# at-cg/PHI

Hardware: AMD Instinct MI355X
Metric: read Gbases/s scored (49-hap MHC graph stand-in synMHC-49); reads resident in HBM, parsing and H2D excluded (higher is better)
Workload: dtype u64

## Files before the change

### phi_amd/csrc/dp_events.hip

```cpp
#include <hip/hip_runtime.h>
#include <type_traits>
#include "phi_kernels.h"

#define NEG (-(1 << 28))
#define NEGK (-(1 << 30))
#define CHK PHI_DP_CHUNK
#define RING PHI_DP_RING
enum { DP_SEQ = 0, DP_ROW = 1, DP_PATH = 2 };

__global__ void __launch_bounds__(256) phi_event_flags_kernel(const int32_t *__restrict__ walk_vtx, int64_t n_entries,
                                                              const int32_t *__restrict__ cvtx, uint8_t *__restrict__ flags)
{
    for (int64_t e = (int64_t)blockIdx.x * blockDim.x + threadIdx.x; e < n_entries; e += (int64_t)gridDim.x * blockDim.x)
        flags[e] = cvtx[walk_vtx[e]] >= 0;
}

__global__ void phi_event_off_kernel(const phi_ent_t *__restrict__ ev_e, int64_t n_ev, const int64_t *__restrict__ walk_off,
                                     int32_t n_walks, int64_t *__restrict__ ev_off)
{
    const int h = blockIdx.x * blockDim.x + threadIdx.x;
    if (h > n_walks) return;
    const int64_t key = walk_off[h];
    int64_t lo = 0, hi = n_ev;
    while (lo < hi) {
// ... 998 lines not shown
        }
        issue(J, min(b + DEPTH, nb - 1));
        __syncthreads();
#pragma unroll
        for (int u = 0; u < U; u++) {
            int32_t best = NEGK;
            if (has_walk) {
                if (live[u]) { const int32_t r = s_diag[p][lx]; if (r > NEGK / 2) best = S[u] + r; }
                {
                    const int32_t o = (live[u] && v[u] == b1[u] && s_n1[p][u][lx] == 1) ? s_b2[p][u][lx] : b1[u];
                    const int32_t kn = s_new[p][lx];
                    if (o > NEGK / 2 && kn > NEGK / 2 && o + kn - dx > best) best = o + kn - dx;
                }
                const int32_t d = max(max(s_part[p][u][0][lx], s_part[p][u][1][lx]), max(s_part[p][u][2][lx], s_part[p][u][3][lx]));
                if (d > NEGK / 2 && d - dx > best) best = d - dx;
                if (with_starts[u]) { const int32_t r = s_start[p][lx]; if (r > NEGK / 2 && r - dx > best) best = r - dx; }
            }
            S[u] = best > NEGK / 2 ? best : NEGK;
        }
    };
    if (x < 64) {
#pragma unroll
        for (int u = 0; u < U; u++) { s_b1[b_lo & 1][u][x] = NONE; s_b2[b_lo & 1][u][x] = NONE; s_n1[b_lo & 1][u][x] = 0; }
    }
    using I0 = std::integral_constant<int, 0>; using I1 = std::integral_constant<int, 1>;
    using I2 = std::integral_constant<int, 2>; using I3 = std::integral_constant<int, 3>;
    issue(I0{}, min(b_lo, nb - 1));
    issue(I1{}, min(b_lo + 1, nb - 1));
    issue(I2{}, min(b_lo + 2, nb - 1));
    issue(I3{}, min(b_lo + 3, nb - 1));
    __syncthreads();
    int32_t b = b_lo;
    for (; b + DEPTH <= nb; b += DEPTH) {
        step(I0{}, b);
        step(I1{}, b + 1);
        step(I2{}, b + 2);
        step(I3{}, b + 3);
    }
    if (b < nb) step(I0{}, b);
    if (b + 1 < nb) step(I1{}, b + 1);
    if (b + 2 < nb) step(I2{}, b + 2);
    if (MODE == 1 && has_walk) {
#pragma unroll
        for (int u = 0; u < U; u++)
            if (unit0 + u <= G.n_walks) seg_row[((int64_t)seg * (G.n_walks + 1) + unit0 + u) * LS + x] = S[u];
    }
}

__global__ void __launch_bounds__(256) phi_seg_chain_kernel(int32_t n_seg, int32_t n_walks, int32_t LS, const int32_t *__restrict__ seg_row,
                                                            int32_t *__restrict__ seg_S)
{
    __shared__ int32_t s_S[256];
    const int x = threadIdx.x;
    int32_t S = NEGK;
    for (int32_t g = 0; g < n_seg; g++) {
        seg_S[(int64_t)g * LS + x] = S;
        s_S[x] = S;
        __syncthreads();
        const int32_t *R = seg_row + (int64_t)g * (n_walks + 1) * LS + x;
        int32_t best = R[(int64_t)n_walks * LS];
#pragma unroll 8
        for (int32_t u = 0; u < n_walks; u++) best = max(best, s_S[u] + R[(int64_t)u * LS]);
        S = best > NEGK / 2 ? best : NEGK;
        __syncthreads();
    }
}

__global__ void __launch_bounds__(256) phi_blk_check_kernel(const int32_t *__restrict__ keys, const int32_t *__restrict__ S, int32_t n_blk,
                                                            int32_t LS, int32_t n_walks, int32_t *__restrict__ bad)
{
    const int64_t n = (int64_t)(n_blk - 1) * LS;
    for (int64_t i = (int64_t)blockIdx.x * blockDim.x + threadIdx.x; i < n; i += (int64_t)gridDim.x * blockDim.x) {
        const int32_t h = (int32_t)(i % LS);
        if (h >= n_walks) continue;
        const int32_t got = keys[i], want = S[i + LS];
        if (got != want && !(got <= NEGK / 2 && want <= NEGK / 2)) { atomicAdd(&bad[0], 1); atomicMin(&bad[1], (int32_t)(i / LS)); }
    }
}

__global__ void __launch_bounds__(256) phi_carry_resolve_kernel(const int32_t *__restrict__ carry, int32_t LS, int32_t b_from, int32_t h,
                                                                int32_t *__restrict__ out)
{
    __shared__ int32_t s_best;
    for (int32_t hi = b_from - 1; hi >= 0; hi -= 256) {
        if (threadIdx.x == 0) s_best = -1;
        __syncthreads();
        const int32_t b = hi - (int32_t)threadIdx.x;
        const int32_t v = b >= 0 ? carry[(int64_t)b * LS + h] : -1;
        if (v >= 0) atomicMax(&s_best, b);
        __syncthreads();
        const int32_t bb = s_best;
        if (bb >= 0) {
            if (b == bb) { out[0] = bb; out[1] = v; }
            return;
        }
        __syncthreads();
    }
    if (threadIdx.x == 0) { out[0] = -1; out[1] = -1; }
}

void phi_launch_blk_classes(hipStream_t st, const PhiBlkClassArgs &G)
{
    if (G.n_blk > 0) hipLaunchKernelGGL(phi_blk_classes_kernel, dim3((unsigned)G.n_blk), dim3(256), 0, st, G);
}
void phi_launch_blk_chain(hipStream_t st, const PhiBlkClassArgs &G, const int32_t *rows, const int32_t *rownew, const int32_t *rowdiag, int32_t *blk_S)
{
    hipLaunchKernelGGL(phi_blk_chain_kernel<0>, dim3(1), dim3(256), 0, st, G, rows, rownew, rowdiag, blk_S, nullptr, nullptr, nullptr);
}
void phi_launch_blk_chain_segments(hipStream_t st, const PhiBlkClassArgs &G, const int32_t *rows, const int32_t *rownew, const int32_t *rowdiag, int32_t *blk_S,
                                   int32_t n_seg, const int32_t *d_seg_lo, int32_t *seg_row, int32_t *seg_S)
{
    const int units = getenv("PHI_DP_CHAIN_UNITS") ? atoi(getenv("PHI_DP_CHAIN_UNITS")) : 3;
// ... 51 lines not shown
```

### phi_amd/csrc/phi_ctx.h

```cpp
#pragma once
#include <stdint.h>
#include <stdarg.h>
#include <stdio.h>
#include <stdlib.h>
#include <algorithm>
#include <atomic>
#include <chrono>
#include <future>
#include <mutex>
#include <string>
#include <thread>
#include <vector>
#include <hip/hip_runtime.h>
#include "../../include/phi_amd.h"
#include "phi_kernels.h"
#include "phi_host_par.h"

struct DevBuf {
    void *p = nullptr;
    size_t cap = 0;
    uint32_t gen = 0;
    template <class T> T *as() const { return reinterpret_cast<T *>(p); }
};

// ... 162 lines not shown
        uint32_t why = 0, first_bad = 0;
    } text;

    struct PhiBamStream {
        bool active = false, failed = false, header_done = false;
        int32_t n_ref = 0;
        uint32_t tile = 0, list_cap = 0, max_tiles = 0, max_rec = 0;
        uint32_t carry_cap = 0, chunk_cap = 0;
        std::vector<unsigned char> h_hdr;
        int64_t fed = 0;
        DevBuf text[2];
        DevBuf bases, roff, sum;
        DevBuf t_first, t_exit, t_status, t_cnt, t_skip, t_list, t_has, t_has_pre, t_use, t_base;
        DevBuf rec_pos, rec_keep, kidx, klen, kseq, krev;
        int slot = 0;
        uint32_t carry_len = 0, carry_at = 0;
        void *h_sum = nullptr;
        hipEvent_t ev_copy = nullptr;
        int64_t one_len = -1;
        int64_t dbg_reads = 0, dbg_bases = 0;
        phi_bam_info info{};
    } bam;

    struct PhiLadder {
        bool collecting = false, have_store = false, have_plan = false;
        int64_t first_ordinal = 0;
        int64_t n_reads = 0, n_bases = 0;
        int64_t one_len = -1;
        DevBuf d_bases, d_off;
        DevBuf d_pbases, d_poff, d_pidx, d_psrc, d_wg, d_tab;
        int64_t band_read0[PHI_LADDER_MAX_LEVELS + 1] = {0}, band_pos[PHI_LADDER_MAX_LEVELS + 1] = {0};
        int32_t scored = 0;
        phi_ladder_info info{};
    } ladder;

    DevBuf d_blk_cnt, d_blk_off, d_flags, d_flags2, d_list, d_list2, d_list3, d_walk_last;
    DevBuf d_sel_off, d_sel_tri;
    DevBuf d_adj_off, d_adj, d_topo_rank, d_cnt_edge, d_walk_err;
    DevBuf d_sa_cnt, d_sa_cur, d_sa_off, d_sa_idx;

    DevBuf d_m_rec, d_m_group, d_g_keys, d_g_rep, d_g_cnt, d_slot_maxcnt, d_slot_multi;
    DevBuf d_a_e1, d_g_off, d_g_span, d_a_weight;
    DevBuf d_dmax, d_bstart, d_top, d_ent, d_word;
    bool dp_dense_ready = false;
    bool dp_events = false;
    int32_t n_k = 0;
    int64_t n_ev = 0;
    std::vector<int32_t> h_cstep, h_kstep;
    std::vector<int32_t> h_k_cut_ok;
    bool dp_blocks = false;
    int32_t n_blk = 0, blk_ring = 1024, blk_max_len = 0;
    std::vector<int32_t> h_blk_lo;
    DevBuf d_blk_lo, d_blk_ev, d_blk_S, d_row_out, d_rowend, d_blk_keys, d_blk_carry, d_cov, d_cov2, d_stepdiff;
    bool dp_cls = false;
    int32_t blk_cls_target = 16;
    bool blk_no_small = false;
    int32_t blk_ls = 64;
    DevBuf d_lane_walk, d_walk_lane, d_coff, d_blk_ncls, d_rownew, d_blk_bad;
    DevBuf d_seg_lo, d_seg_row, d_seg_S;
    DevBuf d_k_rec, d_k_in, d_cvtx, d_ev_e, d_ev_off, d_ev, d_off_end, d_off_start, d_scan_blk, d_scan_blk64, d_scan_blkoff;
    DevBuf d_anchors, d_cov_all, d_cov_w, d_slots, d_slots2, d_segs, d_ctr, d_vmax;
    int64_t n_kept = 0, n_dp = 0;
    bool anchors_host = false;
    PhiAnchorSpan h_kept, h_dp;
    std::vector<PhiAnchorHost> h_dp_own;
    void *h_pin = nullptr;
    size_t h_pin_cap = 0;
    std::future<void> pin_future;
    std::future<int> dp_alloc_future;
    std::vector<uint64_t> h_kept_hash;
    std::vector<int32_t> h_path_vtx, h_path_hap;
    std::vector<int64_t> h_n_minimizers, h_n_anchors;
    phi_result result{};
    bool solved = false;

    bool prof = false;
    std::vector<std::pair<hipEvent_t, hipEvent_t>> prof_events;
    int prof_period = 1;
    uint64_t prof_seq = 0;
    size_t prof_used = 0;
    int64_t prof_bases = 0;
    double prof_ms_done = 0.0;
    int64_t prof_n_done = 0;
};

struct PhiStageTimer {
    bool on;
    const char *what;
    std::chrono::steady_clock::time_point t0;
    explicit PhiStageTimer(const char *w) : on(getenv("PHI_TIMING") != nullptr), what(w), t0(std::chrono::steady_clock::now()) {}
    void lap(const char *stage)
    {
        if (!on) return;
        const auto t1 = std::chrono::steady_clock::now();
        fprintf(stderr, "[phi timing] %s: %-28s %8.3f ms\n", what, stage, std::chrono::duration<double, std::milli>(t1 - t0).count());
        t0 = t1;
    }
};

static inline hipError_t phi_copy_sync(phi_ctx *c, void *dst, const void *src, size_t n, hipMemcpyKind kind)
{
    const hipError_t e = hipMemcpyAsync(dst, src, n, kind, c->stream);
    return e != hipSuccess ? e : hipStreamSynchronize(c->stream);
}
static inline hipError_t phi_memset_sync(phi_ctx *c, void *dst, int v, size_t n)
{
    const hipError_t e = hipMemsetAsync(dst, v, n, c->stream);
// ... 73 lines not shown
```

### phi_amd/csrc/phi_solve.hip

```cpp
#include <stdio.h>
#include <string.h>
#include <algorithm>
#include <map>
#include <set>
#include <unordered_map>
#include "phi_ctx.h"
#include "phi_dev.h"

#define HIPCHK(call) do { int rc_ = phi_hip_check(c, (call), #call); if (rc_) return rc_; } while (0)
#define PHICHK(call) do { int rc_ = (call); if (rc_) return rc_; } while (0)

static bool have_host_walks(const phi_ctx *c) { return (int64_t)c->h_walk_vtx.size() == c->n_entries; }
static int walk_vtx_at(phi_ctx *c, int64_t e, int32_t *v)
{
    if (have_host_walks(c)) { *v = c->h_walk_vtx[(size_t)e]; return PHI_OK; }
    return phi_hip_check(c, phi_copy_sync(c, v, c->d_walk_vtx.as<int32_t>() + e, 4, hipMemcpyDeviceToHost), "walk entry D2H");
}
static int walk_vtx_range(phi_ctx *c, int64_t es, int64_t n, int32_t *dst)
{
    if (have_host_walks(c)) { memcpy(dst, c->h_walk_vtx.data() + es, (size_t)n * 4); return PHI_OK; }
    return phi_hip_check(c, phi_copy_sync(c, dst, c->d_walk_vtx.as<int32_t>() + es, (size_t)n * 4, hipMemcpyDeviceToHost), "walk entries D2H");
}
static int ensure_host_walks(phi_ctx *c)
{
    if (have_host_walks(c)) return PHI_OK;
    if (!c->h_walk_vtx.resize((size_t)c->n_entries)) return phi_fail(c, PHI_ERR_NOMEM, "host allocation failed");
    return phi_hip_check(c, phi_copy_sync(c, c->h_walk_vtx.data(), c->d_walk_vtx.p, (size_t)c->n_entries * 4, hipMemcpyDeviceToHost), "walk entries D2H");
}

struct Seg { int32_t h; int64_t es, ee; };

int phi_host_anchors(phi_ctx *c)
{
    if (c->anchors_host) return PHI_OK;
    const int64_t n = c->n_kept;
    PHICHK(phi_pin_ensure(c, (size_t)std::max<int64_t>(n, 1) * sizeof(PhiAnchorHost)));
    c->h_kept = PhiAnchorSpan{static_cast<PhiAnchorHost *>(c->h_pin), n};
    if (n) HIPCHK(hipMemcpyAsync(c->h_kept.p, c->d_anchors.p, (size_t)n * 12, hipMemcpyDeviceToHost, c->stream));
    HIPCHK(hipStreamSynchronize(c->stream));
    c->h_dp_own.clear();
    c->h_dp = c->h_kept;
    c->anchors_host = true;
    return PHI_OK;
}

static int dp_prepare_blocks(phi_ctx *c, int64_t n_dp)
{
    c->dp_blocks = false;
    c->n_blk = 0;
    c->dp_cls = false;
    if (!c->dp_events || c->n_walks > PHI_DP_EVENT_MAX_WALKS || getenv("PHI_DP_NOBLOCKS") || c->n_k < 4) return PHI_OK;
    const bool cls = c->n_walks > 64;
    c->blk_ls = cls ? 256 : 64;
    const int64_t ne = c->n_entries;
    const int32_t nk = c->n_k;
    PHICHK(phi_dev_ensure(c, c->d_off_end, (size_t)(ne + 3) * 4));
    PHICHK(phi_dev_ensure(c, c->d_off_start, (size_t)(ne + 3) * 4));
    PHICHK(phi_dev_ensure(c, c->d_stepdiff, (size_t)(nk + 2) * 4));
    int32_t *d_a = c->d_off_end.as<int32_t>(), *d_b = c->d_off_start.as<int32_t>();
    HIPCHK(hipMemsetAsync(c->d_stepdiff.p, 0, (size_t)(nk + 2) * 4, c->stream));
    if (getenv("PHI_CUT_COUNTED")) {
        HIPCHK(hipMemsetAsync(d_a, 0, (size_t)(ne + 3) * 4, c->stream));
        phi_launch_cut_cov(c->stream, c->d_a_e1.as<phi_ent_t>(), c->d_g_span.as<uint8_t>(), n_dp, d_a);
        PHICHK(phi_scan(c, d_a, ne + 1, d_b));
        phi_launch_cut_clean(c->stream, d_b, ne, d_a);
    } else {
        phi_launch_cut_clean_direct(c->stream, c->d_g_off.as<int64_t>(), c->d_g_span.as<uint8_t>(), ne, d_a);
    }
    PHICHK(phi_scan(c, d_a, ne + 1, d_b));
    phi_launch_cut_events(c->stream, c->d_ev_e.as<phi_ent_t>(), c->n_ev, c->d_ev_off.as<int64_t>(), c->d_walk_off.as<int64_t>(), c->n_walks,
                          c->d_walk_vtx.as<int32_t>(), c->d_cvtx.as<int32_t>(), d_b, c->d_stepdiff.as<int32_t>());
    std::vector<int32_t> closed((size_t)nk + 2);
    HIPCHK(hipMemcpyAsync(closed.data(), c->d_stepdiff.p, (size_t)(nk + 2) * 4, hipMemcpyDeviceToHost, c->stream));
    HIPCHK(hipStreamSynchronize(c->stream));
    for (int32_t k = 1; k <= nk + 1; k++) closed[(size_t)k] += closed[(size_t)k - 1];
    auto cut_ok = [&](int32_t k) { return k > 0 && k < nk && c->h_k_cut_ok[(size_t)k] && closed[(size_t)k] == 0; };
    if (getenv("PHI_TIMING")) {
        int64_t n_struct = 0, n_both = 0, longest = 0, run = 0, longest_s = 0, run_s = 0;
        for (int32_t k = 1; k < nk; k++) {
            n_struct += c->h_k_cut_ok[(size_t)k] != 0;
            if (cut_ok(k)) { n_both++; run = 0; } else longest = std::max(longest, ++run);
            if (c->h_k_cut_ok[(size_t)k]) run_s = 0; else longest_s = std::max(longest_s, ++run_s);
        }
        fprintf(stderr, "[phi timing] solve: cuts: %lld of %d steps allowed by the graph (longest closed stretch %lld), %lld also clean of anchors (longest closed stretch %lld)\n",
                (long long)n_struct, nk, (long long)longest_s, (long long)n_both, (long long)longest);
    }
    bool placed = false;
    const int32_t rings_walk[] = {256, 1024, 2048}, rings_cls[] = {256, 512};
    const int32_t *rings = cls ? rings_cls : rings_walk;
    const int n_rings = cls ? 2 : 3;
    static_assert(PHI_DP_BLOCK_MAX == 2048, "the largest ring of tops");
    for (int ri = 0; ri < n_rings && !placed; ri++) {
        const int32_t ring = rings[ri];
        if (ring == 256 && c->blk_no_small) continue;
        int64_t target = (int64_t)nk * (c->n_walks + 1) / 4096;
        target = std::max<int64_t>(64, std::min<int64_t>(ring / 2, target));
        if (cls) target = c->blk_cls_target;
        if (const char *e = getenv("PHI_DP_BLOCK_STEPS")) target = std::max(1, std::min(ring, atoi(e)));
        c->h_blk_lo.assign(1, 0);
        bool ok = true;
        for (int32_t start = 0; nk - start > target && ok;) {
            int32_t cut = -1;
            const int32_t hi = (int32_t)std::min<int64_t>((int64_t)start + ring, nk - 1);
            for (int32_t k = (int32_t)(start + target); k <= hi && cut < 0; k++) if (cut_ok(k)) cut = k;
            for (int32_t k = (int32_t)(start + target) - 1; k > start && cut < 0; k--) if (cut_ok(k)) cut = k;
            if (cut < 0) {
                if (nk - start > ring) ok = false;
                break;
            }
            c->h_blk_lo.push_back(cut);
            start = cut;
        }
        if (ok && nk - c->h_blk_lo.back() <= ring) { placed = true; c->blk_ring = ring; }
    }
    if (!placed) return PHI_OK;
    c->h_blk_lo.push_back(nk);
    c->n_blk = (int32_t)c->h_blk_lo.size() - 1;
    if (c->n_blk < 2) { c->n_blk = 0; return PHI_OK; }
    c->blk_max_len = 0;
    for (int32_t b = 0; b < c->n_blk; b++) c->blk_max_len = std::max(c->blk_max_len, c->h_blk_lo[(size_t)b + 1] - c->h_blk_lo[(size_t)b]);
    const size_t nbk = (size_t)c->n_blk, ls = (size_t)c->blk_ls, nrow = cls ? 65 : (size_t)(c->n_walks + 1);
    PHICHK(phi_dev_ensure(c, c->d_blk_lo, (nbk + 1) * 4));
    PHICHK(phi_dev_ensure(c, c->d_blk_ev, nbk * ls * 4));
    PHICHK(phi_dev_ensure(c, c->d_blk_S, nbk * ls * 4));
    PHICHK(phi_dev_ensure(c, c->d_blk_keys, nbk * ls * 4));
    PHICHK(phi_dev_ensure(c, c->d_blk_carry, nbk * ls * 4));
    {
        const uint32_t before = c->d_row_out.gen;
        PHICHK(phi_dev_ensure(c, c->d_row_out, nbk * nrow * 64 * 4));
        if (c->d_row_out.gen != before) HIPCHK(hipMemsetAsync(c->d_row_out.p, 0xC0, c->d_row_out.cap, c->stream));
    }
    PHICHK(phi_dev_ensure(c, c->d_rowend, nbk * nrow * 4));
    if (cls) {
        PHICHK(phi_dev_ensure(c, c->d_lane_walk, nbk * 64 * 4));
        PHICHK(phi_dev_ensure(c, c->d_walk_lane, nbk * ls * 4));
        PHICHK(phi_dev_ensure(c, c->d_coff, nbk * ls * 4));
        PHICHK(phi_dev_ensure(c, c->d_blk_ncls, nbk * 4));
        PHICHK(phi_dev_ensure(c, c->d_rownew, nbk * nrow * 4));
        PHICHK(phi_dev_ensure(c, c->d_rowdiag, nbk * 64 * 4));
        PHICHK(phi_dev_ensure(c, c->d_blk_bad, 64));
    }
    HIPCHK(hipMemcpyAsync(c->d_blk_lo.p, c->h_blk_lo.data(), (nbk + 1) * 4, hipMemcpyHostToDevice, c->stream));
    phi_launch_blk_ev(c->stream, c->d_blk_lo.as<int32_t>(), c->n_blk, c->d_ev_e.as<phi_ent_t>(), c->d_ev_off.as<int64_t>(), c->n_walks,
                      c->d_walk_vtx.as<int32_t>(), c->d_cvtx.as<int32_t>(), c->d_blk_ev.as<int32_t>());
    HIPCHK(hipStreamSynchronize(c->stream));
    c->dp_blocks = true;
    c->dp_cls = cls;
    if (getenv("PHI_TIMING")) fprintf(stderr, "[phi timing] solve: %d compact steps in %d blocks (rings of %d steps)%s\n", nk, c->n_blk, c->blk_ring, cls ? ", rows on class lanes" : "");
    return PHI_OK;
}

struct DpHost {
    std::vector<int32_t> ends, bstart, ent_u, ent_h;
    std::vector<int32_t> rows, rowend, S, keys, carry;
};

static int run_dp(phi_ctx *c, const std::vector<uint8_t> *wgt, DpHost &H, int64_t *value, std::vector<Seg> *segs)
{
    const int64_t n_dp = c->n_dp;
    const int64_t ne = c->n_entries;
    const int32_t nv = c->n_vtx;
    const bool events = c->dp_events;
    const int32_t n_ent = events ? c->n_k : nv;
    PhiStageTimer tr("dp run");
    if (n_dp && wgt) HIPCHK(hipMemcpyAsync(c->d_a_weight.p, wgt->data(), (size_t)n_dp, hipMemcpyHostToDevice, c->stream));
    int32_t *d_dmax = c->d_dmax.as<int32_t>(), *d_bstart = c->d_bstart.as<int32_t>();
    int32_t *d_ent_src = c->d_ent.as<int32_t>(), *d_ent_h = c->d_ent.as<int32_t>() + n_ent;
    if (events) {
        PHICHK(phi_dev_ensure(c, c->d_wpre, (size_t)(n_dp + 1) * 4));
        PHICHK(phi_scan(c, c->d_a_weight.as<uint8_t>(), n_dp, c->d_wpre.as<int32_t>()));
        PhiDpEventArgs A{};
        A.n_k = c->n_k; A.n_walks = c->n_walks; A.n_ev = c->n_ev;
        A.k_rec = c->d_k_rec.as<int32_t>(); A.k_in_packed = c->d_k_in.as<int32_t>();
        A.walk_off = c->d_walk_off.as<int64_t>();
        A.ev_e = c->d_ev_e.as<phi_ent_t>(); A.ev_off = c->d_ev_off.as<int64_t>();
        A.ev = c->d_ev.p;
        A.g_off = c->d_g_off.as<int64_t>(); A.g_span = c->d_g_span.as<uint8_t>(); A.a_weight = c->d_a_weight.as<uint8_t>();
        A.cost = 2 * (c->recombination / 2);
        A.dmax = d_dmax; A.bstart = d_bstart;
        A.tops = c->d_top.as<int32_t>();
        A.ent_src = d_ent_src; A.ent_h = d_ent_h;
        A.err = (uint32_t *)(c->d_scalars.as<uint64_t>() + S_ERR);
        A.q_limit = getenv("PHI_DP_QLIMIT") ? atoi(getenv("PHI_DP_QLIMIT")) : 0;
        phi_launch_dp_event_fill(c->stream, A, c->d_e_out.as<uint8_t>(), c->d_walk_vtx.as<int32_t>(), c->d_cvtx.as<int32_t>(),
                                 c->d_a_e1.as<phi_ent_t>(), c->d_wpre.as<int32_t>(), ne);
        if (tr.on) { (void)hipStreamSynchronize(c->stream); tr.lap("weights + per-run records"); }
        A.lane_stride = c->blk_ls;
        auto keep_whole_chain = [&](uint32_t kerr, uint32_t bit) -> int {
            kerr &= ~(bit | PHI_KERR_DP_QUEUE | PHI_KERR_DP_CLASSES);
            HIPCHK(phi_copy_sync(c, c->d_scalars.as<uint64_t>() + S_ERR, &kerr, 4, hipMemcpyHostToDevice));
            if (bit == PHI_KERR_DP_CLASSES && c->blk_cls_target > 2 && !getenv("PHI_DP_BLOCK_STEPS")) {
                c->blk_cls_target /= 2;
                PHICHK(dp_prepare_blocks(c, n_dp));
                return run_dp(c, wgt, H, value, segs);
            }
            if (bit == PHI_KERR_DP_QUEUE && c->blk_ring <= 256 && !c->blk_no_small) {
                c->blk_no_small = true;
                PHICHK(dp_prepare_blocks(c, n_dp));
                return run_dp(c, wgt, H, value, segs);
            }
            if (getenv("PHI_DP_STRICT")) return phi_fail(c, PHI_ERR_DEVICE, "DP blocks given up (kernel flag %u) under PHI_DP_STRICT", bit);
            c->dp_blocks = false;
            c->dp_cls = false;
            return run_dp(c, wgt, H, value, segs);
        };
        if (c->dp_blocks && c->dp_cls) {
            const int32_t nb = c->n_blk;
            A.n_blk = nb; A.blk_ring = c->blk_ring; A.blk_max_len = c->blk_max_len; A.blk_lo = c->d_blk_lo.as<int32_t>(); A.blk_ev = c->d_blk_ev.as<int32_t>(); A.blk_S = c->d_blk_S.as<int32_t>();
            A.row_out = c->d_row_out.as<int32_t>(); A.rowend_out = c->d_rowend.as<int32_t>(); A.rownew_out = c->d_rownew.as<int32_t>();
            A.rowdiag_out = c->d_rowdiag.as<int32_t>();
            A.blk_keys_out = c->d_blk_keys.as<int32_t>(); A.blk_carry = c->d_blk_carry.as<int32_t>();
            A.lane_walk = c->d_lane_walk.as<int32_t>();
            PhiBlkClassArgs G{};
            G.n_blk = nb; G.n_walks = c->n_walks; G.lane_stride = c->blk_ls;
            G.blk_lo = A.blk_lo; G.blk_ev = A.blk_ev; G.ev_off = A.ev_off; G.walk_off = A.walk_off; G.ev = A.ev;
            G.lane_walk = c->d_lane_walk.as<int32_t>(); G.walk_lane = c->d_walk_lane.as<int32_t>(); G.coff = c->d_coff.as<int32_t>();
            G.blk_ncls = c->d_blk_ncls.as<int32_t>(); G.err = A.err;
            phi_launch_blk_classes(c->stream, G);
            uint32_t kerr = 0;
            if (tr.on) {
                HIPCHK(hipMemcpyAsync(&kerr, c->d_scalars.as<uint64_t>() + S_ERR, 4, hipMemcpyDeviceToHost, c->stream));
                HIPCHK(hipStreamSynchronize(c->stream));
                tr.lap("block classes");
                if (kerr & PHI_KERR_DP_CLASSES) return keep_whole_chain(kerr, PHI_KERR_DP_CLASSES);
            }
            phi_launch_dp_block_rows(c->stream, A);
            if (tr.on) { (void)hipStreamSynchronize(c->stream); tr.lap("block rows"); }
            {
                int32_t n_seg = nb >= 4096 ? std::min<int32_t>(64, nb / 1024) : 0;
                if (const char *e = getenv("PHI_DP_CHAIN_SEGMENTS")) n_seg = std::max(0, std::min(atoi(e), nb));
                if (n_seg >= 2) {
                    std::vector<int32_t> seg_lo((size_t)n_seg + 1);
                    for (int32_t g_ = 0; g_ <= n_seg; g_++) seg_lo[(size_t)g_] = (int32_t)((int64_t)nb * g_ / n_seg);
                    PHICHK(phi_dev_ensure(c, c->d_seg_lo, ((size_t)n_seg + 1) * 4));
                    PHICHK(phi_dev_ensure(c, c->d_seg_row, (size_t)n_seg * (size_t)(c->n_walks + 1) * (size_t)c->blk_ls * 4));
                    PHICHK(phi_dev_ensure(c, c->d_seg_S, (size_t)n_seg * (size_t)c->blk_ls * 4));
                    HIPCHK(phi_copy_sync(c, c->d_seg_lo.p, seg_lo.data(), seg_lo.size() * 4, hipMemcpyHostToDevice));
                    phi_launch_blk_chain_segments(c->stream, G, A.row_out, A.rownew_out, A.rowdiag_out, c->d_blk_S.as<int32_t>(), n_seg,
                                                  c->d_seg_lo.as<int32_t>(), c->d_seg_row.as<int32_t>(), c->d_seg_S.as<int32_t>());
                } else {
                    phi_launch_blk_chain(c->stream, G, A.row_out, A.rownew_out, A.rowdiag_out, c->d_blk_S.as<int32_t>());
                }
                HIPCHK(hipGetLastError());
            }
            if (tr.on) { (void)hipStreamSynchronize(c->stream); tr.lap("block chain"); }
            A.lane_walk = nullptr;
            phi_launch_dp_block_paths_wide(c->stream, A);
            int32_t bad[2] = {0, INT32_MAX};
            HIPCHK(hipMemcpyAsync(c->d_blk_bad.p, bad, 8, hipMemcpyHostToDevice, c->stream));
            phi_launch_blk_check(c->stream, A.blk_keys_out, A.blk_S, nb, c->blk_ls, c->n_walks, c->d_blk_bad.as<int32_t>());
            HIPCHK(hipMemcpyAsync(bad, c->d_blk_bad.p, 8, hipMemcpyDeviceToHost, c->stream));
            HIPCHK(hipMemcpyAsync(&kerr, c->d_scalars.as<uint64_t>() + S_ERR, 4, hipMemcpyDeviceToHost, c->stream));
            HIPCHK(hipStreamSynchronize(c->stream));
            if (tr.on) tr.lap("block paths + check");
            if (kerr & PHI_KERR_DP_CLASSES) return keep_whole_chain(kerr, PHI_KERR_DP_CLASSES);
            if (kerr & PHI_KERR_DP_QUEUE) return keep_whole_chain(kerr, PHI_KERR_DP_QUEUE);
            if (bad[0])
                return phi_fail(c, PHI_ERR_DEVICE, "DP blocks: %d keys leaving blocks (first in block %d) differ from the chained class rows (internal error)", bad[0], bad[1]);
        } else if (c->dp_blocks) {
            const int32_t nb = c->n_blk, nwk = c->n_walks, nrow = nwk + 1;
            A.n_blk = nb; A.blk_ring = c->blk_ring; A.blk_max_len = c->blk_max_len; A.blk_lo = c->d_blk_lo.as<int32_t>(); A.blk_ev = c->d_blk_ev.as<int32_t>(); A.blk_S = c->d_blk_S.as<int32_t>();
            A.row_out = c->d_row_out.as<int32_t>(); A.rowend_out = c->d_rowend.as<int32_t>();
            A.blk_keys_out = c->d_blk_keys.as<int32_t>(); A.blk_carry = c->d_blk_carry.as<int32_t>();
            phi_launch_dp_block_rows(c->stream, A);
            H.rows.resize((size_t)nb * nrow * 64); H.rowend.resize((size_t)nb * nrow);
            HIPCHK(hipMemcpyAsync(H.rows.data(), A.row_out, H.rows.size() * 4, hipMemcpyDeviceToHost, c->stream));
            HIPCHK(hipMemcpyAsync(H.rowend.data(), A.rowend_out, H.rowend.size() * 4, hipMemcpyDeviceToHost, c->stream));
            uint32_t kerr = 0;
            HIPCHK(hipMemcpyAsync(&kerr, c->d_scalars.as<uint64_t>() + S_ERR, 4, hipMemcpyDeviceToHost, c->stream));
            HIPCHK(hipStreamSynchronize(c->stream));
            if (tr.on) tr.lap("block rows");
            if (kerr & PHI_KERR_DP_QUEUE) return keep_whole_chain(kerr, PHI_KERR_DP_QUEUE);
            H.S.assign((size_t)nb * 64, PHI_DP_NEGK);
            std::vector<int64_t> cur(64, PHI_DP_NEGK), nxt(64);
            int64_t end_best = INT64_MIN;
            for (int32_t b = 0; b < nb; b++) {
                for (int h = 0; h < 64; h++) H.S[(size_t)b * 64 + h] = cur[h] > PHI_DP_NEGK / 2 ? (int32_t)cur[h] : PHI_DP_NEGK;
                std::fill(nxt.begin(), nxt.end(), (int64_t)PHI_DP_NEGK);
                for (int32_t j = 0; j <= nwk; j++) {
                    const int64_t base = j == nwk ? 0 : cur[j];
                    if (j < nwk && base <= PHI_DP_NEGK / 2) continue;
                    const int32_t *row = &H.rows[((size_t)b * nrow + j) * 64];
                    for (int32_t h2 = 0; h2 < nwk; h2++)
                        if (row[h2] > PHI_DP_NEGK / 2) nxt[h2] = std::max(nxt[h2], base + row[h2]);
                    const int32_t re = H.rowend[(size_t)b * nrow + j];
                    if (re > -(1 << 27)) end_best = std::max(end_best, base + re);
                }
                cur.swap(nxt);
            }
            HIPCHK(hipMemcpyAsync(c->d_blk_S.p, H.S.data(), H.S.size() * 4, hipMemcpyHostToDevice, c->stream));
            phi_launch_dp_block_paths(c->stream, A);
            H.keys.resize((size_t)nb * 64); H.carry.resize((size_t)nb * 64);
            HIPCHK(hipMemcpyAsync(H.keys.data(), A.blk_keys_out, H.keys.size() * 4, hipMemcpyDeviceToHost, c->stream));
            HIPCHK(hipMemcpyAsync(H.carry.data(), A.blk_carry, H.carry.size() * 4, hipMemcpyDeviceToHost, c->stream));
            HIPCHK(hipMemcpyAsync(&kerr, c->d_scalars.as<uint64_t>() + S_ERR, 4, hipMemcpyDeviceToHost, c->stream));
            HIPCHK(hipStreamSynchronize(c->stream));
            if (kerr & PHI_KERR_DP_QUEUE) return keep_whole_chain(kerr, PHI_KERR_DP_QUEUE);
            for (int32_t b = 0; b + 1 < nb; b++)
                for (int32_t h = 0; h < nwk; h++) {
                    const int32_t want = H.S[(size_t)(b + 1) * 64 + h], got = H.keys[(size_t)b * 64 + h];
                    if (want != got && !(want <= PHI_DP_NEGK / 2 && got <= PHI_DP_NEGK / 2))
                        return phi_fail(c, PHI_ERR_DEVICE, "DP blocks: block %d leaves key %d on walk %d, the chained matrices say %d (internal error)", b, got, h, want);
                }
            (void)end_best;
        } else {
            phi_launch_dp_events(c->stream, A);
        }
    } else {
        PHICHK(phi_dev_ensure(c, c->d_word, (size_t)c->n_entries * 8));
        phi_launch_dp_words(c->stream, c->d_e_out.as<uint8_t>(), c->d_g_off.as<int64_t>(), c->d_g_span.as<uint8_t>(),
                            c->d_a_weight.as<uint8_t>(), ne, c->d_word.as<uint64_t>());
        PhiDpArgs A{};
        A.n_vtx = nv; A.n_walks = c->n_walks;
        A.st_rec = c->d_st_rec.as<int32_t>(); A.st_mask = c->d_st_mask.as<unsigned long long>();
        A.in_packed = c->d_in_packed.as<int32_t>();
        A.walk_off = c->d_walk_off.as<int64_t>();
        A.word = c->d_word.as<uint64_t>();
        A.g_off = c->d_g_off.as<int64_t>(); A.g_span = c->d_g_span.as<uint8_t>(); A.a_weight = c->d_a_weight.as<uint8_t>();
        A.cost = 2 * (c->recombination / 2);
        A.dmax = d_dmax; A.bstart = d_bstart;
        A.tops = c->d_top.as<int32_t>();
        A.ent_src = d_ent_src; A.ent_h = d_ent_h;
        phi_launch_dp(c->stream, A);
    }
    HIPCHK(hipGetLastError());
    H.ends.resize(c->n_walks);
    phi_launch_gather_i32(c->stream, d_dmax, c->d_walk_last.as<phi_ent_t>(), c->n_walks, c->d_list3.as<int32_t>());
    HIPCHK(hipMemcpyAsync(H.ends.data(), c->d_list3.p, (size_t)c->n_walks * 4, hipMemcpyDeviceToHost, c->stream));
    uint32_t kerr = 0;
    if (events) HIPCHK(hipMemcpyAsync(&kerr, c->d_scalars.as<uint64_t>() + S_ERR, 4, hipMemcpyDeviceToHost, c->stream));
    HIPCHK(hipStreamSynchronize(c->stream));
    tr.lap("kernel");
    if (kerr & PHI_KERR_DP_QUEUE) {
        kerr &= ~PHI_KERR_DP_QUEUE;
        HIPCHK(phi_copy_sync(c, c->d_scalars.as<uint64_t>() + S_ERR, &kerr, 4, hipMemcpyHostToDevice));
        if (!c->dp_dense_ready) return phi_fail(c, PHI_ERR_DEVICE, "event DP queue overflow without a dense fallback (internal error)");
        c->dp_events = false;
        return run_dp(c, wgt, H, value, segs);
    }
    bool bulk = false;
    auto fetch_bulk = [&]() -> int {
        H.bstart.resize(ne); H.ent_u.resize(n_ent); H.ent_h.resize(n_ent);
        HIPCHK(hipMemcpyAsync(H.bstart.data(), d_bstart, (size_t)ne * 4, hipMemcpyDeviceToHost, c->stream));
        HIPCHK(hipMemcpyAsync(H.ent_u.data(), d_ent_src, (size_t)n_ent * 4, hipMemcpyDeviceToHost, c->stream));
        HIPCHK(hipMemcpyAsync(H.ent_h.data(), d_ent_h, (size_t)n_ent * 4, hipMemcpyDeviceToHost, c->stream));
        HIPCHK(hipStreamSynchronize(c->stream));
        bulk = true;
        return PHI_OK;
    };

    int32_t bh = -1;
    int64_t best = INT64_MIN;
    for (int32_t h = 0; h < c->n_walks; h++) {
        const int32_t d = H.ends[h];
        if (d > -(1 << 28) && d > best) { best = d; bh = h; }
    }
    if (bh < 0) return phi_fail(c, PHI_ERR_DEVICE, "DP found no s->e path (internal error)");
    *value = best;
    segs->clear();
    int32_t h = bh;
    int64_t e = c->h_walk_off[h + 1] - 1;
    for (int64_t guard = 0; guard <= (int64_t)nv; guard++) {
        if (!bulk && guard == 64) PHICHK(fetch_bulk());
        int32_t bs = 0;
        if (bulk) bs = H.bstart[e];
        else HIPCHK(phi_copy_sync(c, &bs, d_bstart + e, 4, hipMemcpyDeviceToHost));
        if (bs < 0 && c->dp_blocks && events) {
            int32_t vq = 0;
            PHICHK(walk_vtx_at(c, e, &vq));
            const int32_t kq = c->h_cstep[c->h_topo_rank[vq]];
            int32_t b = (int32_t)(std::upper_bound(c->h_blk_lo.begin(), c->h_blk_lo.end(), kq) - c->h_blk_lo.begin()) - 1;
            if (c->dp_cls) {
                int32_t out[2] = {-1, -1};
                phi_launch_carry_resolve(c->stream, c->d_blk_carry.as<int32_t>(), c->blk_ls, b, h, c->d_blk_bad.as<int32_t>() + 2);
                HIPCHK(hipMemcpyAsync(out, c->d_blk_bad.as<int32_t>() + 2, 8, hipMemcpyDeviceToHost, c->stream));
                HIPCHK(hipStreamSynchronize(c->stream));
                bs = out[1];
            } else {
                while (bs < 0 && --b >= 0) bs = H.carry[(size_t)b * 64 + h];
            }
            if (bs < 0) return phi_fail(c, PHI_ERR_DEVICE, "DP backtrack: a carried run has no beginning (internal error)");
        }
        const int64_t es = c->h_walk_off[h] + bs;
        if (es < c->h_walk_off[h] || es > e) return phi_fail(c, PHI_ERR_DEVICE, "DP backtrack left the walk (internal error)");
// ... 259 lines not shown
            int64_t j = i;
            while (j < n_dp && a_e1[j] == a_e1[i]) j++;
            int32_t &m = vmax[c->h_walk_vtx[a_e1[i]]];
            m = std::max<int32_t>(m, (int32_t)std::min<int64_t>(j - i, INT32_MAX));
            i = j;
        }
        int64_t bound = 0;
        for (int32_t m : vmax) bound += m;
        if (bound >= ((int64_t)1 << 27)) return phi_fail(c, PHI_ERR_UNSUPPORTED, "a path could score %lld >= 2^27 anchors", (long long)bound);
    }

    if (tm.on) fprintf(stderr, "[phi timing] solve: class records %lld, matched %lld, kept %lld -> anchors kept %lld, dp %lld\n", (long long)n_rec, (long long)n_matched, (long long)n_kept_rec, (long long)n_kept, (long long)n_dp);
    tm.lap("filter (GPU) + anchors D2H");
    {
        PHICHK(phi_dev_ensure(c, c->d_a_weight, (size_t)std::max<int64_t>(n_dp, 1)));
        PHICHK(phi_dev_ensure(c, c->d_g_off, (size_t)(c->n_entries + 1) * 8));
        if (n_dp && !dev) {
            HIPCHK(hipMemcpyAsync(c->d_a_e1.p, a_e1.data(), (size_t)n_dp * 4, hipMemcpyHostToDevice, c->stream));
            HIPCHK(hipMemcpyAsync(c->d_g_span.p, a_span.data(), (size_t)n_dp, hipMemcpyHostToDevice, c->stream));
        }
        phi_launch_entry_csr(c->stream, c->d_a_e1.as<phi_ent_t>(), n_dp, c->n_entries, c->d_g_off.as<int64_t>());
        if (dev && n_dp >= ((int64_t)1 << 27)) {
            PHICHK(phi_dev_ensure(c, c->d_vmax, (size_t)c->n_vtx * 4));
            HIPCHK(hipMemsetAsync(c->d_vmax.p, 0, (size_t)c->n_vtx * 4, c->stream));
            HIPCHK(hipMemsetAsync(c->d_ctr.p, 0, 8, c->stream));
            phi_launch_vertex_most(c->stream, c->d_g_off.as<int64_t>(), c->n_entries, c->d_walk_vtx.as<int32_t>(), c->d_vmax.as<int32_t>());
            phi_launch_sum_i32(c->stream, c->d_vmax.as<int32_t>(), c->n_vtx, c->d_ctr.as<unsigned long long>());
            unsigned long long bound = 0;
            HIPCHK(hipMemcpyAsync(&bound, c->d_ctr.p, 8, hipMemcpyDeviceToHost, c->stream));
            HIPCHK(hipStreamSynchronize(c->stream));
            if (bound >= (1ull << 27)) return phi_fail(c, PHI_ERR_UNSUPPORTED, "a path could score %llu >= 2^27 anchors", bound);
        }
        HIPCHK(hipStreamSynchronize(c->stream));
        {
            std::vector<phi_ent_t> last(nw);
            for (int32_t h = 0; h < nw; h++) last[h] = (phi_ent_t)(c->h_walk_off[h + 1] - 1);
            PHICHK(phi_dev_ensure(c, c->d_walk_last, (size_t)nw * 4));
            PHICHK(phi_dev_ensure(c, c->d_list3, (size_t)nw * 4));
            HIPCHK(phi_copy_sync(c, c->d_walk_last.p, last.data(), (size_t)nw * 4, hipMemcpyHostToDevice));
        }
        PHICHK(phi_dev_ensure(c, c->d_dmax, (size_t)c->n_entries * 4));
        PHICHK(phi_dev_ensure(c, c->d_bstart, (size_t)c->n_entries * 4));
        if (c->dp_events) {
            const int64_t ne1 = c->n_entries + 1;
            PHICHK(phi_dev_ensure(c, c->d_off_end, (size_t)(ne1 + 2) * 4));
            PHICHK(phi_dev_ensure(c, c->d_off_start, (size_t)(ne1 + 2) * 4));
            PHICHK(phi_dev_ensure(c, c->d_ev, (size_t)std::max<int64_t>(c->n_ev, 1) * 48));
        }
        PHICHK(phi_dev_ensure(c, c->d_top, (size_t)c->n_vtx * 5 * 4));
        PHICHK(phi_dev_ensure(c, c->d_ent, (size_t)c->n_vtx * 2 * 4));
    }

    c->blk_no_small = false;
    c->blk_cls_target = 16;
    PHICHK(dp_prepare_blocks(c, n_dp));
    tm.lap("DP inputs");
    const int64_t cost = 2 * (int64_t)(c->recombination / 2);
    const int64_t n_ids = c->n_unique;
    std::vector<int32_t> sa_off, sa_idx;
    if (!dev) { sa_off.assign((size_t)n_ids + 1, 0); sa_idx.resize((size_t)std::max<int64_t>(n_dp, 1)); }
    const bool dp_is_kept = dev || (c->h_dp.p == c->h_kept.p && c->h_dp.size() == c->h_kept.size());
    auto build_csr = [&](bool to_host_too) -> int {
        const uint32_t *tri = d_tri;
        PHICHK(phi_dev_ensure(c, c->d_sa_cnt, (size_t)(n_ids + 1) * 4));
        PHICHK(phi_dev_ensure(c, c->d_sa_cur, (size_t)(n_ids + 1) * 4));
        PHICHK(phi_dev_ensure(c, c->d_sa_off, (size_t)(n_ids + 2) * 4));
        PHICHK(phi_dev_ensure(c, c->d_sa_idx, (size_t)n_dp * 4));
        HIPCHK(hipMemsetAsync(c->d_sa_cnt.p, 0, (size_t)(n_ids + 1) * 4, c->stream));
        HIPCHK(hipMemsetAsync(c->d_sa_cur.p, 0, (size_t)(n_ids + 1) * 4, c->stream));
        phi_launch_csr_count(c->stream, tri, n_dp, n_ids, c->d_sa_cnt.as<int32_t>(), (uint32_t *)scalar(c, S_ERR));
        PHICHK(phi_scan(c, c->d_sa_cnt.as<int32_t>(), n_ids, c->d_sa_off.as<int32_t>()));
        phi_launch_csr_scatter(c->stream, tri, n_dp, n_ids, c->d_sa_off.as<int32_t>(), c->d_sa_cur.as<int32_t>(), c->d_sa_idx.as<int32_t>());
        phi_launch_csr_sort(c->stream, c->d_sa_off.as<int32_t>(), n_ids, c->d_sa_idx.as<int32_t>());
        int32_t total = 0;
        if (to_host_too) {
            sa_off.resize((size_t)n_ids + 1); sa_idx.resize((size_t)std::max<int64_t>(n_dp, 1));
            HIPCHK(hipMemcpyAsync(sa_off.data(), c->d_sa_off.p, (size_t)(n_ids + 1) * 4, hipMemcpyDeviceToHost, c->stream));
            HIPCHK(hipMemcpyAsync(sa_idx.data(), c->d_sa_idx.p, (size_t)n_dp * 4, hipMemcpyDeviceToHost, c->stream));
        }
        HIPCHK(hipMemcpyAsync(&total, c->d_sa_off.as<int32_t>() + n_ids, 4, hipMemcpyDeviceToHost, c->stream));
        uint32_t kerr = 0;
        HIPCHK(hipMemcpyAsync(&kerr, scalar(c, S_ERR), 4, hipMemcpyDeviceToHost, c->stream));
        HIPCHK(hipStreamSynchronize(c->stream));
        if ((kerr & PHI_KERR_CSR_ID) || total != (int32_t)n_dp)
            return phi_fail(c, PHI_ERR_DEVICE, "minimiser id out of range (internal error)");
        return PHI_OK;
    };
    if (dev) {
    } else if (dp_is_kept && n_dp > 0) {
        PHICHK(build_csr(true));
    } else {
        for (const PhiAnchorHost &a : c->h_dp) {
            if ((int64_t)a.slot >= n_ids) return phi_fail(c, PHI_ERR_DEVICE, "minimiser id out of range (internal error)");
            sa_off[a.slot + 1]++;
        }
        for (int64_t i = 0; i < n_ids; i++) sa_off[i + 1] += sa_off[i];
        std::vector<int32_t> cur(sa_off.begin(), sa_off.end() - 1);
        for (int64_t i = 0; i < n_dp; i++) sa_idx[cur[c->h_dp[i].slot]++] = (int32_t)i;
    }
    struct Span {
        const int32_t *p; int32_t n;
        const int32_t *begin() const { return p; }
        const int32_t *end() const { return p + n; }
        int32_t operator[](int32_t i) const { return p[i]; }
    };
    auto anchors_of = [&](uint32_t s) { return Span{sa_idx.data() + sa_off[s], sa_off[s + 1] - sa_off[s]}; };
    auto clusters_of = [&](uint32_t slot) {
        const Span idx = anchors_of(slot);
// ... 281 lines not shown
```

Measured before the change: 456.3.

## Route small-panel DP rows onto class lanes and model chain segment count

For panels of 64 or fewer walks, the block DP can now run rows on class lanes when n_k*n_walks exceeds a work threshold. If class placement fails it falls back to walk rows, and it uses the narrow block-paths kernel when n_walks is at most 64. The chain segment count now comes from a small cost model instead of a fixed rule, and segment bounds are uploaded only when that count changes. The walk-end gather is folded into the existing block-path sync to save one stream synchronization. The risks are extra retry paths and a heuristic cost model that may pick poor segmentations.

```diff
diff --git a/phi_amd/csrc/dp_events.hip b/phi_amd/csrc/dp_events.hip
--- a/phi_amd/csrc/dp_events.hip
+++ b/phi_amd/csrc/dp_events.hip
@@ -1074,12 +1074,14 @@
 {
     __shared__ int32_t s_S[256];
     const int x = threadIdx.x;
+    const bool in_row = x < LS;
+    const int xr = in_row ? x : 0;
     int32_t S = NEGK;
     for (int32_t g = 0; g < n_seg; g++) {
-        seg_S[(int64_t)g * LS + x] = S;
+        if (in_row) seg_S[(int64_t)g * LS + x] = S;
         s_S[x] = S;
         __syncthreads();
-        const int32_t *R = seg_row + (int64_t)g * (n_walks + 1) * LS + x;
+        const int32_t *R = seg_row + (int64_t)g * (n_walks + 1) * LS + xr;
         int32_t best = R[(int64_t)n_walks * LS];
 #pragma unroll 8
         for (int32_t u = 0; u < n_walks; u++) best = max(best, s_S[u] + R[(int64_t)u * LS]);
diff --git a/phi_amd/csrc/phi_ctx.h b/phi_amd/csrc/phi_ctx.h
--- a/phi_amd/csrc/phi_ctx.h
+++ b/phi_amd/csrc/phi_ctx.h
@@ -238,7 +238,11 @@
     int32_t n_blk = 0, blk_ring = 1024, blk_max_len = 0;
     std::vector<int32_t> h_blk_lo;
     DevBuf d_blk_lo, d_blk_ev, d_blk_S, d_row_out, d_rowend, d_blk_keys, d_blk_carry, d_cov, d_cov2, d_stepdiff;
+#define PHI_DP_CLASS_MIN_WORK 300000
+#define PHI_DP_CHAIN_RESIDENT 768
     bool dp_cls = false;
+    bool blk_no_cls = false;
+    int32_t seg_lo_n = 0;
     int32_t blk_cls_target = 16;
     bool blk_no_small = false;
     int32_t blk_ls = 64;
diff --git a/phi_amd/csrc/phi_solve.hip b/phi_amd/csrc/phi_solve.hip
--- a/phi_amd/csrc/phi_solve.hip
+++ b/phi_amd/csrc/phi_solve.hip
@@ -44,14 +44,39 @@
     return PHI_OK;
 }
 
+static bool dp_rows_on_class_lanes(const phi_ctx *c)
+{
+    if (const char *e = getenv("PHI_DP_ROWS")) {
+        if (!strcmp(e, "class")) return true;
+        if (!strcmp(e, "walk")) return false;
+    }
+    if (getenv("PHI_DP_BLOCK_STEPS")) return false;
+    return (int64_t)c->n_k * c->n_walks >= PHI_DP_CLASS_MIN_WORK;
+}
+
+static int32_t dp_chain_segments(int32_t nb, int32_t n_walks)
+{
+    const double groups = (double)((n_walks + 1 + 2) / 3);
+    double best = 1.2 * nb;
+    int32_t best_n = 0;
+    for (int32_t n = 2; n <= 64 && n * 4 <= nb; n++) {
+        const double len = (double)nb / n, wg = n * groups;
+        const double rounds = wg <= PHI_DP_CHAIN_RESIDENT ? 1.0 : wg / PHI_DP_CHAIN_RESIDENT + 0.5;
+        const double t = rounds * len * 2.7 + n * 0.07 * n_walks + len * 0.9 + 10.0;
+        if (t < best) { best = t; best_n = n; }
+    }
+    return best_n;
+}
+
 static int dp_prepare_blocks(phi_ctx *c, int64_t n_dp)
 {
     c->dp_blocks = false;
     c->n_blk = 0;
     c->dp_cls = false;
+    c->seg_lo_n = 0;
     if (!c->dp_events || c->n_walks > PHI_DP_EVENT_MAX_WALKS || getenv("PHI_DP_NOBLOCKS") || c->n_k < 4) return PHI_OK;
-    const bool cls = c->n_walks > 64;
-    c->blk_ls = cls ? 256 : 64;
+    bool cls = c->n_walks > 64 || (!c->blk_no_cls && dp_rows_on_class_lanes(c));
+    c->blk_ls = c->n_walks > 64 ? 256 : 64;
     const int64_t ne = c->n_entries;
     const int32_t nk = c->n_k;
     PHICHK(phi_dev_ensure(c, c->d_off_end, (size_t)(ne + 3) * 4));
@@ -85,11 +110,12 @@
         fprintf(stderr, "[phi timing] solve: cuts: %lld of %d steps allowed by the graph (longest closed stretch %lld), %lld also clean of anchors (longest closed stretch %lld)\n",
                 (long long)n_struct, nk, (long long)longest_s, (long long)n_both, (long long)longest);
     }
+    static_assert(PHI_DP_BLOCK_MAX == 2048, "the largest ring of tops");
+    auto place = [&]() -> bool {
     bool placed = false;
     const int32_t rings_walk[] = {256, 1024, 2048}, rings_cls[] = {256, 512};
     const int32_t *rings = cls ? rings_cls : rings_walk;
     const int n_rings = cls ? 2 : 3;
-    static_assert(PHI_DP_BLOCK_MAX == 2048, "the largest ring of tops");
     for (int ri = 0; ri < n_rings && !placed; ri++) {
         const int32_t ring = rings[ri];
         if (ring == 256 && c->blk_no_small) continue;
@@ -113,10 +139,20 @@
         }
         if (ok && nk - c->h_blk_lo.back() <= ring) { placed = true; c->blk_ring = ring; }
     }
+    if (placed) {
+        c->h_blk_lo.push_back(nk);
+        c->n_blk = (int32_t)c->h_blk_lo.size() - 1;
+        if (c->n_blk < 2) { c->n_blk = 0; placed = false; }
+    }
+    return placed;
+    };
+    bool placed = place();
+    if (!placed && cls && c->n_walks <= 64) {
+        c->blk_no_cls = true;
+        cls = false;
+        placed = place();
+    }
     if (!placed) return PHI_OK;
-    c->h_blk_lo.push_back(nk);
-    c->n_blk = (int32_t)c->h_blk_lo.size() - 1;
-    if (c->n_blk < 2) { c->n_blk = 0; return PHI_OK; }
     c->blk_max_len = 0;
     for (int32_t b = 0; b < c->n_blk; b++) c->blk_max_len = std::max(c->blk_max_len, c->h_blk_lo[(size_t)b + 1] - c->h_blk_lo[(size_t)b]);
     const size_t nbk = (size_t)c->n_blk, ls = (size_t)c->blk_ls, nrow = cls ? 65 : (size_t)(c->n_walks + 1);
@@ -163,6 +199,7 @@
     const bool events = c->dp_events;
     const int32_t n_ent = events ? c->n_k : nv;
     PhiStageTimer tr("dp run");
+    bool have_ends = false;
     if (n_dp && wgt) HIPCHK(hipMemcpyAsync(c->d_a_weight.p, wgt->data(), (size_t)n_dp, hipMemcpyHostToDevice, c->stream));
     int32_t *d_dmax = c->d_dmax.as<int32_t>(), *d_bstart = c->d_bstart.as<int32_t>();
     int32_t *d_ent_src = c->d_ent.as<int32_t>(), *d_ent_h = c->d_ent.as<int32_t>() + n_ent;
@@ -200,6 +237,12 @@
                 return run_dp(c, wgt, H, value, segs);
             }
             if (getenv("PHI_DP_STRICT")) return phi_fail(c, PHI_ERR_DEVICE, "DP blocks given up (kernel flag %u) under PHI_DP_STRICT", bit);
+            if (c->dp_cls && c->n_walks <= 64) {
+                c->blk_no_cls = true;
+                c->blk_no_small = false;
+                PHICHK(dp_prepare_blocks(c, n_dp));
+                return run_dp(c, wgt, H, value, segs);
+            }
             c->dp_blocks = false;
             c->dp_cls = false;
             return run_dp(c, wgt, H, value, segs);
@@ -227,15 +270,19 @@
             phi_launch_dp_block_rows(c->stream, A);
             if (tr.on) { (void)hipStreamSynchronize(c->stream); tr.lap("block rows"); }
             {
-                int32_t n_seg = nb >= 4096 ? std::min<int32_t>(64, nb / 1024) : 0;
+                int32_t n_seg = dp_chain_segments(nb, c->n_walks);
                 if (const char *e = getenv("PHI_DP_CHAIN_SEGMENTS")) n_seg = std::max(0, std::min(atoi(e), nb));
                 if (n_seg >= 2) {
-                    std::vector<int32_t> seg_lo((size_t)n_seg + 1);
-                    for (int32_t g_ = 0; g_ <= n_seg; g_++) seg_lo[(size_t)g_] = (int32_t)((int64_t)nb * g_ / n_seg);
                     PHICHK(phi_dev_ensure(c, c->d_seg_lo, ((size_t)n_seg + 1) * 4));
                     PHICHK(phi_dev_ensure(c, c->d_seg_row, (size_t)n_seg * (size_t)(c->n_walks + 1) * (size_t)c->blk_ls * 4));
                     PHICHK(phi_dev_ensure(c, c->d_seg_S, (size_t)n_seg * (size_t)c->blk_ls * 4));
-                    HIPCHK(phi_copy_sync(c, c->d_seg_lo.p, seg_lo.data(), seg_lo.size() * 4, hipMemcpyHostToDevice));
+                    if (c->seg_lo_n != n_seg) {
+                        std::vector<int32_t> seg_lo((size_t)n_seg + 1);
+                        for (int32_t g_ = 0; g_ <= n_seg; g_++) seg_lo[(size_t)g_] = (int32_t)((int64_t)nb * g_ / n_seg);
+                        HIPCHK(phi_copy_sync(c, c->d_seg_lo.p, seg_lo.data(), seg_lo.size() * 4, hipMemcpyHostToDevice));
+                        c->seg_lo_n = n_seg;
+                    }
+                    if (tr.on) fprintf(stderr, "[phi timing] dp run: chain over %d blocks in %d segments\n", nb, n_seg);
                     phi_launch_blk_chain_segments(c->stream, G, A.row_out, A.rownew_out, A.rowdiag_out, c->d_blk_S.as<int32_t>(), n_seg,
                                                   c->d_seg_lo.as<int32_t>(), c->d_seg_row.as<int32_t>(), c->d_seg_S.as<int32_t>());
                 } else {
@@ -245,12 +292,17 @@
             }
             if (tr.on) { (void)hipStreamSynchronize(c->stream); tr.lap("block chain"); }
             A.lane_walk = nullptr;
-            phi_launch_dp_block_paths_wide(c->stream, A);
+            if (c->n_walks <= 64) phi_launch_dp_block_paths(c->stream, A);
+            else phi_launch_dp_block_paths_wide(c->stream, A);
             int32_t bad[2] = {0, INT32_MAX};
             HIPCHK(hipMemcpyAsync(c->d_blk_bad.p, bad, 8, hipMemcpyHostToDevice, c->stream));
             phi_launch_blk_check(c->stream, A.blk_keys_out, A.blk_S, nb, c->blk_ls, c->n_walks, c->d_blk_bad.as<int32_t>());
             HIPCHK(hipMemcpyAsync(bad, c->d_blk_bad.p, 8, hipMemcpyDeviceToHost, c->stream));
             HIPCHK(hipMemcpyAsync(&kerr, c->d_scalars.as<uint64_t>() + S_ERR, 4, hipMemcpyDeviceToHost, c->stream));
+            H.ends.resize(c->n_walks);
+            phi_launch_gather_i32(c->stream, d_dmax, c->d_walk_last.as<phi_ent_t>(), c->n_walks, c->d_list3.as<int32_t>());
+            HIPCHK(hipMemcpyAsync(H.ends.data(), c->d_list3.p, (size_t)c->n_walks * 4, hipMemcpyDeviceToHost, c->stream));
+            have_ends = true;
             HIPCHK(hipStreamSynchronize(c->stream));
             if (tr.on) tr.lap("block paths + check");
             if (kerr & PHI_KERR_DP_CLASSES) return keep_whole_chain(kerr, PHI_KERR_DP_CLASSES);
@@ -324,12 +376,14 @@
         phi_launch_dp(c->stream, A);
     }
     HIPCHK(hipGetLastError());
-    H.ends.resize(c->n_walks);
-    phi_launch_gather_i32(c->stream, d_dmax, c->d_walk_last.as<phi_ent_t>(), c->n_walks, c->d_list3.as<int32_t>());
-    HIPCHK(hipMemcpyAsync(H.ends.data(), c->d_list3.p, (size_t)c->n_walks * 4, hipMemcpyDeviceToHost, c->stream));
     uint32_t kerr = 0;
-    if (events) HIPCHK(hipMemcpyAsync(&kerr, c->d_scalars.as<uint64_t>() + S_ERR, 4, hipMemcpyDeviceToHost, c->stream));
-    HIPCHK(hipStreamSynchronize(c->stream));
+    if (!have_ends) {
+        H.ends.resize(c->n_walks);
+        phi_launch_gather_i32(c->stream, d_dmax, c->d_walk_last.as<phi_ent_t>(), c->n_walks, c->d_list3.as<int32_t>());
+        HIPCHK(hipMemcpyAsync(H.ends.data(), c->d_list3.p, (size_t)c->n_walks * 4, hipMemcpyDeviceToHost, c->stream));
+        if (events) HIPCHK(hipMemcpyAsync(&kerr, c->d_scalars.as<uint64_t>() + S_ERR, 4, hipMemcpyDeviceToHost, c->stream));
+        HIPCHK(hipStreamSynchronize(c->stream));
+    }
     tr.lap("kernel");
     if (kerr & PHI_KERR_DP_QUEUE) {
         kerr &= ~PHI_KERR_DP_QUEUE;
@@ -695,8 +749,8 @@
     }
 
     c->blk_no_small = false;
-    c->blk_cls_target = 16;
-    PHICHK(dp_prepare_blocks(c, n_dp));
+    c->blk_no_cls = false;
+    c->blk_cls_target = 16;    PHICHK(dp_prepare_blocks(c, n_dp));
     tm.lap("DP inputs");
     const int64_t cost = 2 * (int64_t)(c->recombination / 2);
     const int64_t n_ids = c->n_unique;
diff --git a/profiles/dp_rows_route.py b/profiles/dp_rows_route.py
--- /dev/null
+++ b/profiles/dp_rows_route.py
@@ -0,0 +1,134 @@
+import argparse
+import json
+import os
+import re
+import sys
+import tempfile
+import time
+
+import numpy as np
+import torch
+
+ROOT = os.path.dirname(os.path.dirname(os.path.abspath(__file__)))
+sys.path.insert(0, ROOT)
+import phi_amd
+from phi_amd import synth
+
+PANELS = [8, 16, 24, 32, 49]
+ROUTES = {"walk": {"PHI_DP_ROWS": "walk"}, "class": {"PHI_DP_ROWS": "class"}, "default": {}}
+LAP = re.compile(r"\[phi timing\] dp run: (.*?)\s+([0-9.]+) ms")
+
+
+def set_arrays(ctx, A, **kw):
+    return ctx.set_graph(A["seq_concat"], A["seq_off"], A["adj_off"], A["adj"], A["walk_off"], A["walk_vtx"], A.get("top_rank"), **kw)
+
+
+class Env:
+    def __init__(self, env):
+        self.env = env
+
+    def __enter__(self):
+        self.old = {k: os.environ.get(k) for k in self.env}
+        os.environ.update(self.env)
+
+    def __exit__(self, *exc):
+        for k, v in self.old.items():
+            if v is None:
+                os.environ.pop(k, None)
+            else:
+                os.environ[k] = v
+
+
+def timed_laps(ctx):
+    with tempfile.TemporaryFile() as f, Env({"PHI_TIMING": "1"}):
+        sys.stderr.flush()
+        saved = os.dup(2)
+        os.dup2(f.fileno(), 2)
+        try:
+            ctx.solve()
+        finally:
+            os.dup2(saved, 2)
+            os.close(saved)
+        f.seek(0)
+        text = f.read().decode(errors="replace")
+    laps, runs = {}, 0
+    for name, ms in LAP.findall(text):
+        laps[name] = laps.get(name, 0.0) + float(ms)
+        runs += name == "weights + per-run records"
+    runs = max(runs, 1)
+    chain = re.search(r"chain over (\d+) blocks in (\d+) segments", text)
+    return {k: v / runs for k, v in laps.items()}, runs, int(chain.group(2)) if chain else 0
+
+
+def measure(ctx, stream, routes, repeats):
+    rows = {name: {"solve_s": []} for name in routes}
+    for rep in range(repeats + 1):
+        for name, env in routes.items():
+            with Env(env):
+                stream.synchronize()
+                t0 = time.perf_counter()
+                res = ctx.solve()
+                dt = time.perf_counter() - t0
+                info = ctx.solve_stats()
+            if rep:
+                rows[name]["solve_s"].append(dt)
+            rows[name].update(objective=int(res["objective"]), optimal=int(res["optimal"]), n_dp_runs=int(res["n_dp_runs"]), **info)
+    for name, env in routes.items():
+        with Env(env):
+            laps, runs, n_seg = timed_laps(ctx)
+        r = rows[name]
+        r["solve_s_median"] = float(np.median(r["solve_s"]))
+        r["dp_run_laps_ms"], r["dp_run_ms"], r["chain_segments"] = laps, sum(laps.values()), n_seg
+    assert len({(r["objective"], r["optimal"]) for r in rows.values()}) == 1, rows
+    return rows
+
+
+def main():
+    ap = argparse.ArgumentParser()
+    ap.add_argument("--repeats", type=int, default=7)
+    ap.add_argument("--out", default=os.path.join(ROOT, "profiles", "dp_rows_route.json"))
+    a = ap.parse_args()
+    stream = torch.cuda.Stream()
+    torch.cuda.set_stream(stream)
+
+    def fresh():
+        ctx = phi_amd.Context(0)
+        ctx.set_params(k=31, w=25, threshold=1.0, recombination=100)
+        ctx.set_stream(stream.cuda_stream)
+        ctx.set_solve_budget(16)
+        return ctx
+    out = {"repeats": a.repeats, "graphs": []}
+    gk, rk = synth.CONFIGS["C2"]
+    g = synth.make_graph(**gk)
+    bases, off, truth = synth.make_reads(g, **rk)
+    A = g.arrays()
+    order = list(dict.fromkeys([int(h) for h in truth["walks"]] + list(range(g.n_walks))))
+    for n in PANELS:
+        ctx = fresh()
+        mask = np.zeros(g.n_walks, np.uint8)
+        mask[order[:n]] = 1
+        set_arrays(ctx, A, keep=mask)
+        ctx.add_reads((bases, off))
+        routes = dict(ROUTES)
+        if n == g.n_walks:
+            routes["class, blocks of 32"] = {"PHI_DP_ROWS": "class", "PHI_DP_BLOCK_STEPS": "32"}
+        rows = measure(ctx, stream, routes, a.repeats)
+        out["graphs"].append({"graph": f"C2 panel of {n}", "n_walks": n, "n_steps": rows["walk"]["n_steps"], "routes": rows})
+        print(n, {k: (round(v["solve_s_median"] * 1e3, 3), round(v["dp_run_ms"], 3), v["dp_mode"], v["n_blocks"]) for k, v in rows.items()}, flush=True)
+        ctx.close()
+    g = synth.graph_from_gfa(os.path.join(ROOT, "tests", "golden", "data", "MHC_4.gfa.gz"))
+    bases, off, _ = synth.make_reads(g, coverage=1.0, seed=4102, n_mosaic=2)
+    ctx = fresh()
+    set_arrays(ctx, g.arrays())
+    ctx.add_reads((bases, off))
+    rows = measure(ctx, stream, ROUTES, a.repeats)
+    out["graphs"].append({"graph": "C1syn", "n_walks": g.n_walks, "n_steps": rows["walk"]["n_steps"], "routes": rows})
+    print("C1syn", {k: (round(v["solve_s_median"] * 1e3, 3), round(v["dp_run_ms"], 3), v["dp_mode"], v["n_blocks"]) for k, v in rows.items()}, flush=True)
+    ctx.close()
+    with open(a.out, "w") as f:
+        json.dump(out, f, indent=1)
+        f.write("\n")
+
+
+if __name__ == "__main__":
+    main()
```

New measurement: 456.1, median of 3. No clear change (-0.0%).
